# eriklindernoren/PyTorch-GAN

Hardware: NVIDIA H100
Metric: DCGAN 64x64 images/sec (full G+D step) (higher is better)
Workload: dtype tf32 (fp32 storage, fp32 accumulate)

## Files before the change

include/b200gan.h:

```cpp
#ifndef B200GAN_H
#define B200GAN_H

#include <stddef.h>
#include <stdint.h>

#ifdef __cplusplus
extern "C" {
#endif

#define B200GAN_VERSION 100

enum {
  B200GAN_OK = 0,
  B200GAN_E_UNSUPPORTED = -1,
  B200GAN_E_BAD_ARG = -2,
  B200GAN_E_CUDA = -3,
  B200GAN_E_ARCH = -4
};

enum { B200GAN_ACT_NONE = 0, B200GAN_ACT_LRELU = 1, B200GAN_ACT_RELU = 2, B200GAN_ACT_TANH = 3,
       B200GAN_ACT_SIGMOID = 4 };

enum { B200GAN_ALGO_AUTO = 0,
       B200GAN_ALGO_SIMT = 1,
       B200GAN_ALGO_TC = 2 };

enum { B200GAN_PAD_ZERO = 0, B200GAN_PAD_REFLECT = 1 };

enum {
  B200GAN_PACK_SIMT_FPROP = 0,
  B200GAN_PACK_SIMT_DGRAD = 1,
  B200GAN_PACK_TC_FPROP = 2,
  B200GAN_PACK_TC_DGRAD = 3,
  B200GAN_PACK_TC_FPROP_UP2 = 4,
  B200GAN_PACK_TC_DGRAD_UP2 = 5
};

typedef struct b200gan_conv_geom {
  int32_t N, H, W, C;
  int32_t K;
  int32_t R, S;
  int32_t stride;
  int32_t pad_t, pad_l, pad_b, pad_r;
  int32_t pad_mode;
  int32_t up;
  int32_t transposed;
  int32_t P, Q;
} b200gan_conv_geom;

typedef struct b200gan_epilogue {
  const float *bias;
  int32_t act;
  float slope;
  const float *chan_scale;
  double *stats;
  int32_t stats_per_sample;
  int32_t round_tf32;
} b200gan_epilogue;

int b200gan_version(void);
const char *b200gan_last_error(void);
int b200gan_check_device(void);

size_t b200gan_packed_weight_floats(const b200gan_conv_geom *g, int pack);
int b200gan_pack_weights(const b200gan_conv_geom *g, int pack, const float *w, float *packed,
                         void *stream);

typedef struct b200gan_pack_job {
  const float *w;
  float *packed;
  b200gan_conv_geom geom;
  int32_t pack;
} b200gan_pack_job;
int b200gan_pack_weights_multi(const b200gan_pack_job *jobs, int32_t count, void *stream);

int b200gan_conv2d_supported(const b200gan_conv_geom *g, int pass, int algo);

int b200gan_conv2d_fprop(const b200gan_conv_geom *g, const b200gan_epilogue *ep, const float *x,
                         const float *packed, float *y, int algo, void *stream);

size_t b200gan_conv2d_dgrad_workspace_floats(const b200gan_conv_geom *g, int algo);
int b200gan_conv2d_dgrad(const b200gan_conv_geom *g, const float *dy, const float *packed,
                         float *dx, float *workspace, int algo, void *stream);

size_t b200gan_conv2d_wgrad_workspace_floats(const b200gan_conv_geom *g, int algo);
int b200gan_conv2d_wgrad(const b200gan_conv_geom *g, const float *x, const float *dy, float *dw,
                         float *db, float *workspace, int algo, void *stream);
int b200gan_conv2d_wgrad_fused_bias(const b200gan_conv_geom *g, const float *x, const float *dy, float *dw,
                                    float *db, float *workspace, int algo, void *stream);

int b200gan_epilogue_bwd(const float *dy, const float *y, const float *chan_scale, int32_t act,
                         float slope, int64_t n, int32_t K, int64_t PQ, int32_t round_tf32,
                         float *dz, void *stream);

int b200gan_bias_grad(const float *dy, const float *y, const float *chan_scale, int32_t act, float slope,
                      int64_t rows, int32_t K, int64_t PQ, float *db, void *stream);

typedef struct b200gan_norm_desc {
  int32_t N, HW, C;
  int32_t per_sample;
  float eps;
  float momentum;
  int32_t act;
  float slope;
  int32_t round_tf32;
} b200gan_norm_desc;

int b200gan_norm_stats(const b200gan_norm_desc *d, const float *x, double *stats, void *stream);
int b200gan_norm_finalize(const b200gan_norm_desc *d, double *stats, const float *gamma,
                          const float *beta, float *mean_rstd, float *scale_shift,
                          float *running_mean, float *running_var, int64_t *num_batches_tracked,
                          void *stream);
int b200gan_norm_apply(const b200gan_norm_desc *d, const float *x, const float *scale_shift,
                       float *y, void *stream);
int b200gan_norm_bwd(const b200gan_norm_desc *d, const float *dy, const float *x, const float *y,
                     const float *mean_rstd, const float *scale_shift, const float *gamma, double *sums, float *dx,
                     float *dgamma_dbeta, void *stream);

int b200gan_conv2d_dgrad_norm_supported(const b200gan_conv_geom *g);
int b200gan_conv2d_dgrad_norm(const b200gan_conv_geom *g, const b200gan_norm_desc *d, const float *dy,
                              const float *packed, const float *x, const float *mean_rstd, const float *scale_shift,
                              double *sums, float *dx, void *stream);
int b200gan_norm_bwd_from_sums(const b200gan_norm_desc *d, const float *dy, const float *x, const float *mean_rstd,
                               const float *scale_shift, const float *gamma, double *sums, float *dx,
                               float *dgamma_dbeta, void *stream);

typedef struct b200gan_tail_desc {
  int32_t N, H, W, C;
  int32_t K;
  int32_t act_mid;
  float slope;
  int32_t act_out;
} b200gan_tail_desc;
int b200gan_tail_supported(const b200gan_tail_desc *d);
int b200gan_tail_fprop(const b200gan_tail_desc *d, const float *a, const float *scale_shift, const float *w,
                       const float *bias, float *out, void *stream);
size_t b200gan_tail_bwd_workspace_bytes(const b200gan_tail_desc *d);
int b200gan_tail_bwd(const b200gan_tail_desc *d, const float *a, const float *mean_rstd, const float *scale_shift,
                     const float *w, const float *g, void *workspace, float *da, float *dgamma_dbeta, float *dw,
                     float *db, int32_t round_tf32, void *stream);

int b200gan_nchw_to_nhwc(const float *x, float *y, int32_t N, int32_t C, int32_t HW, void *stream);
int b200gan_nhwc_to_nchw(const float *x, float *y, int32_t N, int32_t C, int32_t HW, void *stream);
int b200gan_upsample2x_fwd(const float *x, float *y, int32_t N, int32_t H, int32_t W, int32_t C,
                           void *stream);
int b200gan_upsample2x_bwd(const float *dy, float *dx, int32_t N, int32_t H, int32_t W, int32_t C,
                           void *stream);
int b200gan_pad2d_fwd(const float *x, float *y, int32_t N, int32_t H, int32_t W, int32_t C,
                      int32_t pad_t, int32_t pad_l, int32_t pad_b, int32_t pad_r, int32_t mode,
                      int32_t round_tf32, void *stream);
int b200gan_pad2d_bwd(const float *dy, float *dx, int32_t N, int32_t H, int32_t W, int32_t C,
                      int32_t pad_t, int32_t pad_l, int32_t pad_b, int32_t pad_r, int32_t mode,
                      void *stream);
int b200gan_act_fwd(const float *x, const float *mask, int32_t mask_per_channel, int32_t act,
                    float slope, int64_t n, int32_t C, int64_t HW, float *y, void *stream);

typedef struct b200gan_mlp_critic_desc {
  int32_t N, Din, H1, H2;
  float slope;
} b200gan_mlp_critic_desc;
int b200gan_mlp_critic_fwd(const b200gan_mlp_critic_desc *d, const float *x, const float *W1,
                           const float *b1, const float *W2, const float *b2, const float *W3,
                           const float *b3, float *out, float *m1, float *a1, float *m2, float *a2,
                           void *stream);
size_t b200gan_mlp_critic_bwd_workspace_floats(const b200gan_mlp_critic_desc *d);
int b200gan_mlp_critic_bwd(const b200gan_mlp_critic_desc *d, const float *dout, const float *x,
                           const float *W1, const float *W2, const float *W3, const float *m1,
                           const float *a1, const float *m2, const float *a2, float *dx, float *dW1,
                           float *db1, float *dW2, float *db2, float *dW3, float *db3, float *U1,
                           float *U2, float *workspace, void *stream);
size_t b200gan_mlp_critic_dbwd_workspace_floats(const b200gan_mlp_critic_desc *d);
int b200gan_mlp_critic_dbwd(const b200gan_mlp_critic_desc *d, const float *u, const float *dout,
// ... 85 lines not shown
```

pytorch-gan_b200/b200gan/_lib.py:

```python
import ctypes
import os

_HERE = os.path.dirname(os.path.abspath(__file__))
LIB_PATH = os.path.join(_HERE, "libb200gan.so")

c_i32, c_i64, c_f32, c_f64 = ctypes.c_int32, ctypes.c_int64, ctypes.c_float, ctypes.c_double
c_vp, c_sz = ctypes.c_void_p, ctypes.c_size_t

ACT_NONE, ACT_LRELU, ACT_RELU, ACT_TANH, ACT_SIGMOID = 0, 1, 2, 3, 4
ALGO_AUTO, ALGO_SIMT, ALGO_TC = 0, 1, 2
PAD_ZERO, PAD_REFLECT = 0, 1
PACK_SIMT_FPROP, PACK_SIMT_DGRAD, PACK_TC_FPROP, PACK_TC_DGRAD, PACK_TC_FPROP_UP2, PACK_TC_DGRAD_UP2 = range(6)


class ConvGeom(ctypes.Structure):
    _fields_ = [(n, c_i32) for n in (
        "N", "H", "W", "C", "K", "R", "S", "stride", "pad_t", "pad_l", "pad_b", "pad_r",
        "pad_mode", "up", "transposed", "P", "Q")]

    def key(self):
        return tuple(getattr(self, n) for n, _ in self._fields_)


class Epilogue(ctypes.Structure):
    _fields_ = [("bias", c_vp), ("act", c_i32), ("slope", c_f32), ("chan_scale", c_vp),
                ("stats", c_vp), ("stats_per_sample", c_i32), ("round_tf32", c_i32)]


class NormDesc(ctypes.Structure):
    _fields_ = [("N", c_i32), ("HW", c_i32), ("C", c_i32), ("per_sample", c_i32), ("eps", c_f32),
                ("momentum", c_f32), ("act", c_i32), ("slope", c_f32), ("round_tf32", c_i32)]


class MlpCriticDesc(ctypes.Structure):
    _fields_ = [("N", c_i32), ("Din", c_i32), ("H1", c_i32), ("H2", c_i32), ("slope", c_f32)]


MLP_GEN_MAX_LAYERS, MLP_GEN_MAX_WIDTH, MLP_GEN_MAX_N = 8, 8192, 8192


class MlpGenDesc(ctypes.Structure):
    _fields_ = [("L", c_i32), ("N", c_i32), ("width", c_i32 * (MLP_GEN_MAX_LAYERS + 1)),
                ("has_norm", c_i32 * MLP_GEN_MAX_LAYERS), ("slope", c_f32), ("eps", c_f32), ("momentum", c_f32)] + [
        (n, c_vp * MLP_GEN_MAX_LAYERS)
        for n in ("W", "b", "gamma", "beta", "running_mean", "running_var", "num_batches_tracked")]


class MlpGenGrads(ctypes.Structure):
    _fields_ = [(n, c_vp * MLP_GEN_MAX_LAYERS) for n in ("dW", "db", "dgamma", "dbeta")]


class PackJob(ctypes.Structure):
    _fields_ = [("w", c_vp), ("packed", c_vp), ("geom", ConvGeom), ("pack", c_i32)]


class NbBn(ctypes.Structure):
    _fields_ = [("stats", c_vp), ("gamma", c_vp), ("beta", c_vp), ("eps", c_f32), ("count", c_f64), ("groups", c_i32),
                ("reserved", c_i32)]


class TailDesc(ctypes.Structure):
    _fields_ = [("N", c_i32), ("H", c_i32), ("W", c_i32), ("C", c_i32), ("K", c_i32), ("act_mid", c_i32),
                ("slope", c_f32), ("act_out", c_i32)]


class AdamTensor(ctypes.Structure):
    _fields_ = [("p", c_vp), ("g", c_vp), ("m", c_vp), ("v", c_vp), ("n", c_i64)]


_P = ctypes.POINTER
SIGNATURES = {
    "b200gan_version": (c_i32, []),
    "b200gan_last_error": (ctypes.c_char_p, []),
    "b200gan_check_device": (c_i32, []),
    "b200gan_packed_weight_floats": (c_sz, [_P(ConvGeom), c_i32]),
    "b200gan_pack_weights": (c_i32, [_P(ConvGeom), c_i32, c_vp, c_vp, c_vp]),
    "b200gan_pack_weights_multi": (c_i32, [_P(PackJob), c_i32, c_vp]),
    "b200gan_conv2d_supported": (c_i32, [_P(ConvGeom), c_i32, c_i32]),
    "b200gan_conv2d_fprop": (c_i32, [_P(ConvGeom), _P(Epilogue), c_vp, c_vp, c_vp, c_i32, c_vp]),
    "b200gan_conv2d_dgrad_workspace_floats": (c_sz, [_P(ConvGeom), c_i32]),
    "b200gan_conv2d_dgrad": (c_i32, [_P(ConvGeom), c_vp, c_vp, c_vp, c_vp, c_i32, c_vp]),
    "b200gan_conv2d_wgrad_workspace_floats": (c_sz, [_P(ConvGeom), c_i32]),
    "b200gan_conv2d_wgrad": (c_i32, [_P(ConvGeom), c_vp, c_vp, c_vp, c_vp, c_vp, c_i32, c_vp]),
    "b200gan_conv2d_wgrad_fused_bias": (c_i32, [_P(ConvGeom), c_vp, c_vp, c_vp, c_vp, c_vp, c_i32, c_vp]),
    "b200gan_epilogue_bwd": (c_i32, [c_vp, c_vp, c_vp, c_i32, c_f32, c_i64, c_i32, c_i64, c_i32, c_vp, c_vp]),
    "b200gan_bias_grad": (c_i32, [c_vp, c_vp, c_vp, c_i32, c_f32, c_i64, c_i32, c_i64, c_vp, c_vp]),
    "b200gan_norm_stats": (c_i32, [_P(NormDesc), c_vp, c_vp, c_vp]),
    "b200gan_norm_finalize": (c_i32, [_P(NormDesc), c_vp, c_vp, c_vp, c_vp, c_vp, c_vp, c_vp, c_vp, c_vp]),
    "b200gan_norm_apply": (c_i32, [_P(NormDesc), c_vp, c_vp, c_vp, c_vp]),
    "b200gan_norm_bwd": (c_i32, [_P(NormDesc), c_vp, c_vp, c_vp, c_vp, c_vp, c_vp, c_vp, c_vp, c_vp, c_vp]),
    "b200gan_conv2d_dgrad_norm_supported": (c_i32, [_P(ConvGeom)]),
    "b200gan_conv2d_dgrad_norm": (c_i32, [_P(ConvGeom), _P(NormDesc)] + [c_vp] * 8),
    "b200gan_norm_bwd_from_sums": (c_i32, [_P(NormDesc)] + [c_vp] * 9),
    "b200gan_tail_supported": (c_i32, [_P(TailDesc)]),
    "b200gan_tail_fprop": (c_i32, [_P(TailDesc), c_vp, c_vp, c_vp, c_vp, c_vp, c_vp]),
    "b200gan_tail_bwd_workspace_bytes": (c_sz, [_P(TailDesc)]),
    "b200gan_tail_bwd": (c_i32, [_P(TailDesc)] + [c_vp] * 10 + [c_i32, c_vp]),
    "b200gan_nchw_to_nhwc": (c_i32, [c_vp, c_vp, c_i32, c_i32, c_i32, c_vp]),
    "b200gan_nhwc_to_nchw": (c_i32, [c_vp, c_vp, c_i32, c_i32, c_i32, c_vp]),
    "b200gan_upsample2x_fwd": (c_i32, [c_vp, c_vp, c_i32, c_i32, c_i32, c_i32, c_vp]),
    "b200gan_upsample2x_bwd": (c_i32, [c_vp, c_vp, c_i32, c_i32, c_i32, c_i32, c_vp]),
    "b200gan_pad2d_fwd": (c_i32, [c_vp, c_vp] + [c_i32] * 10 + [c_vp]),
    "b200gan_pad2d_bwd": (c_i32, [c_vp, c_vp] + [c_i32] * 9 + [c_vp]),
    "b200gan_act_fwd": (c_i32, [c_vp, c_vp, c_i32, c_i32, c_f32, c_i64, c_i32, c_i64, c_vp, c_vp]),
    "b200gan_mlp_critic_fwd": (c_i32, [_P(MlpCriticDesc)] + [c_vp] * 13),
    "b200gan_mlp_critic_bwd_workspace_floats": (c_sz, [_P(MlpCriticDesc)]),
    "b200gan_mlp_critic_bwd": (c_i32, [_P(MlpCriticDesc)] + [c_vp] * 20),
    "b200gan_mlp_critic_dbwd_workspace_floats": (c_sz, [_P(MlpCriticDesc)]),
    "b200gan_mlp_critic_dbwd": (c_i32, [_P(MlpCriticDesc)] + [c_vp] * 15),
    "b200gan_critic_step_workspace_floats": (c_sz, [_P(MlpCriticDesc)]),
    "b200gan_critic_step_mlp": (c_i32, [_P(MlpCriticDesc), c_f32] + [c_vp] * 18),
    "b200gan_mlp_gen_saved_floats": (c_sz, [_P(MlpGenDesc)]),
    "b200gan_mlp_gen_workspace_floats": (c_sz, [_P(MlpGenDesc)]),
    "b200gan_mlp_gen_fwd": (c_i32, [_P(MlpGenDesc)] + [c_vp] * 5),
    "b200gan_mlp_gen_bwd": (c_i32, [_P(MlpGenDesc)] + [c_vp] * 5 + [_P(MlpGenGrads), c_vp, c_vp]),
    "b200gan_nb_supported": (c_i32, [_P(ConvGeom)]),
    "b200gan_nb_groups_supported": (c_i32, [_P(ConvGeom), c_i32]),
    "b200gan_nb_fprop": (c_i32, [_P(ConvGeom), _P(NbBn), c_vp, c_vp, c_vp, c_f32, c_vp, c_vp, c_vp, c_i32, c_f32, c_vp,
                                 c_vp, c_vp, c_i32, c_vp]),
    "b200gan_nb_dz": (c_i32, [c_i32, c_i64, c_i32, c_vp, c_vp, c_vp, c_i32, c_f32, _P(NbBn), c_vp, c_vp, c_vp, c_vp]),
    "b200gan_nb_wgrad_workspace_floats": (c_sz, [_P(ConvGeom)]),
    "b200gan_nb_wgrad": (c_i32, [_P(ConvGeom), _P(NbBn), c_vp, c_vp, c_vp, c_vp, c_vp]),
    "b200gan_nb_dgrad": (c_i32, [_P(ConvGeom), c_vp, c_vp, _P(NbBn), c_vp, c_vp, c_vp, c_vp]),
    "b200gan_nb_tail_fwd": (c_i32, [c_i32, c_i32, c_i32, _P(NbBn), c_vp, c_vp, c_vp, c_f32, c_vp, c_vp, c_i32, c_vp]),
    "b200gan_nb_tail_bwd": (c_i32, [c_i32, c_i32, c_i32, _P(NbBn), c_vp, c_vp, c_i32, c_vp, c_vp, c_vp]),
    "b200gan_linear1_fwd": (c_i32, [c_vp, c_vp, c_vp, c_vp, c_i32, c_i32, c_i32, c_vp]),
    "b200gan_linear1_bwd": (c_i32, [c_vp] * 7 + [c_i32, c_i32, c_i32, c_vp]),
    "b200gan_bce_fwd": (c_i32, [c_vp, c_vp, c_vp, c_i64, c_vp]),
    "b200gan_bce_bwd": (c_i32, [c_vp, c_vp, c_vp, c_vp, c_i64, c_vp]),
    "b200gan_adam_multi": (c_i32, [_P(AdamTensor), c_i32, c_f64, c_f64, c_f64, c_f64, c_f32, c_vp, c_vp]),
}

_lib = None


def load():
    global _lib
    if _lib is not None:
        return _lib
    if not os.path.exists(LIB_PATH):
        raise RuntimeError(
            f"{LIB_PATH} is missing: run `python pytorch-gan_b200/build.py` (or __graft_entry__.build()). "
            "b200gan has no CPU / cuDNN fallback.")
    lib = ctypes.CDLL(LIB_PATH)
    for name, (res, args) in SIGNATURES.items():
        fn = getattr(lib, name)
        fn.restype = res
        fn.argtypes = args
    _lib = lib
    return lib


CALLS = 0


def check(rc, what=""):
    global CALLS
    CALLS += 1
    if rc != 0:
        msg = load().b200gan_last_error().decode("utf-8", "replace")
        raise RuntimeError(f"libb200gan {what} failed (code {rc}): {msg}")
```

pytorch-gan_b200/csrc/wgrad_tc.cu:

```cuda
#include "tc_common.cuh"
#include <stdlib.h>

namespace b200gan {

constexpr int WG_THREADS = 384;
constexpr int WG_MAX_JOBS = 52;
constexpr int WG_PIX = 32;
constexpr int WG_CHUNK_BYTES = WG_PIX * 128;

struct WgJob {
  int16_t s_dc, d_dc;
  int8_t s_da, d_da;
  int8_t s_dw, s_dh;
  int8_t db;
  int8_t pad_;
};

struct WgParams {
  WgJob jobs[WG_MAX_JOBS];
  int32_t njobs;
  int32_t bw_log2, bh_log2;
  int32_t tiles_w, tiles_h, N;
  int32_t imgs_per_box;
  int32_t tiles_total, tiles_per_split;
  int32_t s_is_a;
  int32_t mtiles, ntiles;
  int32_t ldn;
  int32_t mtotal;
  float *partial;
  float *db;
};

template <int NB, int STAGES>
struct WgSmem {
  static constexpr int A_BYTES = 4 * WG_CHUNK_BYTES;
  static constexpr int B_BYTES = (NB / 32) * WG_CHUNK_BYTES;
  static constexpr int STAGE_BYTES = A_BYTES + B_BYTES;
  static constexpr int RING = STAGES * STAGE_BYTES;
  static constexpr int T_BYTES = NB * 128;
  static constexpr int STAGING = (NB / 32) * 16384;
  static constexpr int MAIN = RING + 2 * T_BYTES > STAGING ? RING + 2 * T_BYTES : STAGING;
  static constexpr int TOTAL = MAIN + 1024 + 256;
  static_assert(TOTAL <= 232448, "wgrad_tc_kernel: shared memory");
};

__device__ __forceinline__ void wg_consumers_sync() { asm volatile("bar.sync 1, 256;" ::: "memory"); }

__device__ __forceinline__ int wg_kpos(int p) { return (p & ~7) | ((p & 7) >> 1) | ((p & 1) << 2); }

template <int NB, int STAGES>
__global__ void __launch_bounds__(WG_THREADS, 1)
wgrad_tc_kernel(const __grid_constant__ CUtensorMap tmX, const __grid_constant__ CUtensorMap tmY,
                const __grid_constant__ CUtensorMap tmP, const __grid_constant__ WgParams p) {
  using L = WgSmem<NB, STAGES>;
  extern __shared__ uint8_t smem_raw[];
  uint8_t *smem = reinterpret_cast<uint8_t *>((reinterpret_cast<uintptr_t>(smem_raw) + 1023) & ~(uintptr_t)1023);
  uint64_t *full = reinterpret_cast<uint64_t *>(smem + L::MAIN);
  uint64_t *empty = full + STAGES;

  const int warp = threadIdx.x >> 5, lane = threadIdx.x & 31;
  const int split = blockIdx.x, job = blockIdx.y;
  const int mt = blockIdx.z / p.ntiles, nt = blockIdx.z % p.ntiles;
  const int t_begin = split * p.tiles_per_split;
  int t_end = t_begin + p.tiles_per_split;
  if (t_end > p.tiles_total) t_end = p.tiles_total;
  const int iters = t_end - t_begin;

  if (threadIdx.x == 0) {
    tma_prefetch_desc(&tmX);
    tma_prefetch_desc(&tmY);
    for (int s = 0; s < STAGES; ++s) {
      mbar_init(&full[s], 1);
      mbar_init(&empty[s], 256);
    }
    fence_barrier_init();
  }
  __syncthreads();

  if (warp < 4) {
    setmaxnreg_dec<40>();
    if (warp == 0 && lane == 0) {
      const WgJob jb = p.jobs[job];
      const CUtensorMap *mapA = p.s_is_a ? &tmX : &tmY;
      const CUtensorMap *mapB = p.s_is_a ? &tmY : &tmX;
      const int a_dc = p.s_is_a ? jb.s_dc : jb.d_dc, a_da = p.s_is_a ? jb.s_da : jb.d_da;
      const int a_dw = p.s_is_a ? jb.s_dw : 0, a_dh = p.s_is_a ? jb.s_dh : 0;
      const int b_dc = p.s_is_a ? jb.d_dc : jb.s_dc, b_da = p.s_is_a ? jb.d_da : jb.s_da;
      const int b_dw = p.s_is_a ? 0 : jb.s_dw, b_dh = p.s_is_a ? 0 : jb.s_dh;
      int stage = 0;
      uint32_t phase = 0;
      for (int it = 0; it < iters; ++it) {
        int t = t_begin + it;
        const int tw = t % p.tiles_w;
        t /= p.tiles_w;
        const int th = t % p.tiles_h;
        const int n = (t / p.tiles_h) * p.imgs_per_box;
        const int w0 = tw << p.bw_log2, h0 = th << p.bh_log2;
        mbar_wait(&empty[stage], phase ^ 1);
        uint8_t *sa = smem + stage * L::STAGE_BYTES;
        uint8_t *sb = sa + L::A_BYTES;
        mbar_arrive_expect_tx(&full[stage], L::STAGE_BYTES);
#pragma unroll
        for (int c = 0; c < 4; ++c)
          tma_load_5d(sa + c * WG_CHUNK_BYTES, mapA, &full[stage], a_dc + (mt * 4 + c) * 32, w0 + a_dw, a_da,
                      h0 + a_dh, n);
#pragma unroll
        for (int c = 0; c < NB / 32; ++c)
          tma_load_5d(sb + c * WG_CHUNK_BYTES, mapB, &full[stage], b_dc + (nt * (NB / 32) + c) * 32, w0 + b_dw, b_da,
                      h0 + b_dh, n);
        if (++stage == STAGES) {
          stage = 0;
          phase ^= 1;
        }
      }
    }
  } else {
    setmaxnreg_inc<232>();
    if (iters == 0) return;
    const int ct = threadIdx.x - 128;
    const int half = ct >> 7;
    const int tp = ct & 31, tq = ct >> 5;
    const int tk = wg_kpos(tp);
    const int wq = tq & 3;
    const int ac = 16 * (wq & 1) + (lane >> 2), ap = 2 * (lane & 3);
    const int abase = (2 * half + (wq >> 1)) * WG_CHUNK_BYTES + ap * 128 + (ac & 3) * 4;
    const uint32_t aoff[4] = {
        (uint32_t)(abase + ((((ac >> 2)) ^ ap) << 4)),
        (uint32_t)(abase + ((((ac >> 2) + 2) ^ ap) << 4)),
        (uint32_t)(abase + 128 + ((((ac >> 2)) ^ (ap + 1)) << 4)),
        (uint32_t)(abase + 128 + ((((ac >> 2) + 2) ^ (ap + 1)) << 4))};
    float acc[NB / 2];
    const bool db_job = p.db != nullptr && p.jobs[job].db;
    const bool dbA = db_job && !p.s_is_a && nt == 0;
    const bool dbB = db_job && p.s_is_a && mt == 0;
    float dsa0 = 0.f, dsa1 = 0.f;
    float dsb[NB <= 64 ? NB / 8 : 1];
#pragma unroll
    for (int i = 0; i < (NB <= 64 ? NB / 8 : 1); ++i) dsb[i] = 0.f;
    int stage = 0;
    uint32_t phase = 0;
    auto prepare = [&](int it, uint32_t(&fa)[16]) {
      uint8_t *tb = smem + L::RING + (it & 1) * L::T_BYTES;
      mbar_wait(&full[stage], phase);
      wg_consumers_sync();
      const uint8_t *src = smem + stage * L::STAGE_BYTES;
#pragma unroll
      for (int k = 0; k < WG_PIX / 8; ++k)
#pragma unroll
        for (int j = 0; j < 4; ++j) fa[4 * k + j] = *reinterpret_cast<const uint32_t *>(src + aoff[j] + k * 1024);
      if (dbA) {
#pragma unroll
        for (int k = 0; k < WG_PIX / 8; ++k) {
          dsa0 += __uint_as_float(fa[4 * k]) + __uint_as_float(fa[4 * k + 2]);
          dsa1 += __uint_as_float(fa[4 * k + 1]) + __uint_as_float(fa[4 * k + 3]);
        }
      }
#pragma unroll
      for (int c = 0; c < NB / 32; ++c) {
        const float4 v = *reinterpret_cast<const float4 *>(src + L::A_BYTES + c * WG_CHUNK_BYTES + tp * 128 +
                                                           ((tq ^ (tp & 7)) << 4));
        const float e[4] = {v.x, v.y, v.z, v.w};
        if constexpr (NB <= 64) {
          if (dbB) {
#pragma unroll
            for (int i = 0; i < 4; ++i) dsb[4 * c + i] += e[i];
          }
        }
#pragma unroll
        for (int i = 0; i < 4; ++i) {
          const int r = c * 32 + tq * 4 + i;
          *reinterpret_cast<float *>(tb + r * 128 + (((tk >> 2) ^ (r & 7)) << 4) + (tk & 3) * 4) = e[i];
        }
      }
      mbar_arrive(&empty[stage]);
      fence_proxy_async();
      wg_consumers_sync();
      if (++stage == STAGES) {
        stage = 0;
        phase ^= 1;
      }
    };
    auto mma = [&](int it, const uint32_t(&fa)[16]) {
      const uint32_t sb = smem_u32(smem + L::RING + (it & 1) * L::T_BYTES);
      wgmma_fence();
#pragma unroll
      for (int k = 0; k < WG_PIX / 8; ++k)
        wgmma_tf32_rs<NB>(acc, fa + 4 * k, gmma_desc_sw128(sb + k * 32), (it > 0 || k > 0) ? 1u : 0u);
      wgmma_commit();
    };
    uint32_t fa0[16], fa1[16];
    prepare(0, fa0);
#pragma unroll 1
    for (int it = 0; it < iters; it += 2) {
      mma(it, fa0);
      if (it + 1 < iters) prepare(it + 1, fa1);
      wgmma_wait<0>();
      if (it + 1 < iters) {
        mma(it + 1, fa1);
        if (it + 2 < iters) prepare(it + 2, fa0);
        wgmma_wait<0>();
      }
    }
    wgmma_wait<0>();
    wgmma_fence_regs<NB / 2>(acc);
    if (dbA) {
      dsa0 += __shfl_xor_sync(0xffffffffu, dsa0, 1);
      dsa1 += __shfl_xor_sync(0xffffffffu, dsa1, 1);
      dsa0 += __shfl_xor_sync(0xffffffffu, dsa0, 2);
      dsa1 += __shfl_xor_sync(0xffffffffu, dsa1, 2);
      if ((lane & 3) == 0) {
        const int ch = (mt * 4 + 2 * half + (wq >> 1)) * 32 + ac;
        atomicAdd(p.db + ch, dsa0);
        atomicAdd(p.db + ch + 8, dsa1);
      }
    }
    if constexpr (NB <= 64) {
      if (dbB) {
#pragma unroll
        for (int i = 0; i < NB / 8; ++i) {
          float s = dsb[i];
#pragma unroll
          for (int o = 16; o > 0; o >>= 1) s += __shfl_xor_sync(0xffffffffu, s, o);
          if (lane == 0) atomicAdd(p.db + nt * NB + (i >> 2) * 32 + tq * 4 + (i & 3), s);
        }
      }
    }
    wg_consumers_sync();
    store_acc_sw128<NB>(smem, acc, half * 64);
    fence_proxy_async();
    wg_consumers_sync();
    if (ct == 0) {
      const int row0 = job * p.mtotal + mt * 128;
#pragma unroll 1
      for (int c = 0; c < NB; c += 32) tma_reduce_add_2d(&tmP, smem + (c >> 5) * 16384, nt * NB + c, row0);
      tma_store_commit_and_wait_read();
    }
  }
}

struct WgReduceP {
  int32_t K, C, R, S, njobs, s_is_a, up2, transposed;
  int32_t mtotal, ldn;
};
__device__ __forceinline__ bool up2_contrib(int r, int a, int d) {
  if (a == 0) return d == 0 ? r == 0 : r >= 1;
  return d == 0 ? r <= 1 : r == 2;
}
__global__ void wgrad_reduce_kernel(const float *__restrict__ partial, float *__restrict__ dw, WgReduceP p) {
  int64_t total = (int64_t)p.K * p.C * p.R * p.S;
  for (int64_t i = (int64_t)blockIdx.x * blockDim.x + threadIdx.x; i < total;
       i += (int64_t)gridDim.x * blockDim.x) {
    int c = (int)(i % p.C);
    int64_t t = i / p.C;
    int k = (int)(t % p.K);
    t /= p.K;
    int s = (int)(t % p.S), r = (int)(t / p.S);
    const int sch = p.transposed ? k : c;
    const int dch = p.transposed ? c : k;
    int64_t elem = p.s_is_a ? (int64_t)sch * p.ldn + dch : (int64_t)dch * p.ldn + sch;
    int64_t job_stride = (int64_t)p.mtotal * p.ldn;
    const float *base = partial + elem;
    float acc = 0.f;
    if (!p.up2) {
      acc = __ldg(base + (int64_t)(r * p.S + s) * job_stride);
    } else {
      for (int j = 0; j < 16; ++j) {
        int ph = j >> 2, tp = j & 3;
        if (up2_contrib(r, ph >> 1, tp >> 1) && up2_contrib(s, ph & 1, tp & 1)) acc += __ldg(base + j * job_stride);
      }
    }
    const int64_t o = p.transposed ? (((int64_t)c * p.K + k) * p.R + r) * p.S + s
                                   : (((int64_t)k * p.C + c) * p.R + r) * p.S + s;
    dw[o] = acc;
  }
}


constexpr int WR_COL = 32, WR_ROW = 8, WR_TAPS = 16;
__global__ void __launch_bounds__(256)
wgrad_reduce_tile_kernel(const float *__restrict__ partial, float *__restrict__ dw, WgReduceP p) {
  __shared__ float s[WR_ROW][WR_COL][WR_TAPS + 1];
  const int RS = p.R * p.S;
  const int tin = p.up2 ? 16 : RS;
  const bool col_is_k = (p.s_is_a != 0) != (p.transposed != 0);
  const int ncol = col_is_k ? p.K : p.C, nrow = col_is_k ? p.C : p.K;
  const int tiles_col = (ncol + WR_COL - 1) / WR_COL;
  const int col0 = (blockIdx.x % tiles_col) * WR_COL, row0 = (blockIdx.x / tiles_col) * WR_ROW;
  const int64_t job_stride = (int64_t)p.mtotal * p.ldn;
  const int tid = threadIdx.x;
  for (int e = tid; e < WR_COL * WR_ROW * tin; e += 256) {
    const int cl = e % WR_COL, rw = (e / WR_COL) % WR_ROW, j = e / (WR_COL * WR_ROW);
    float v = 0.f;
    if (col0 + cl < ncol && row0 + rw < nrow) v = __ldg(partial + j * job_stride + (int64_t)(row0 + rw) * p.ldn + col0 + cl);
    s[rw][cl][j] = v;
  }
  __syncthreads();
  const bool col_is_b = col_is_k == (p.transposed != 0);
  const int nb = p.transposed ? p.K : p.C;
  for (int e = tid; e < WR_COL * WR_ROW * RS; e += 256) {
    const int t = e % RS;
    int cl, rw;
    if (col_is_b) { cl = (e / RS) % WR_COL; rw = e / (RS * WR_COL); }
    else          { rw = (e / RS) % WR_ROW; cl = e / (RS * WR_ROW); }
    const int col = col0 + cl, row = row0 + rw;
    if (col >= ncol || row >= nrow) continue;
    float acc;
    if (!p.up2) {
      acc = s[rw][cl][t];
    } else {
      const int r = t / 3, q = t % 3;
      acc = 0.f;
#pragma unroll
      for (int j = 0; j < 16; ++j) {
        const int ph = j >> 2, tp = j & 3;
        if (up2_contrib(r, ph >> 1, tp >> 1) && up2_contrib(q, ph & 1, tp & 1)) acc += s[rw][cl][j];
      }
    }
    const int a = col_is_b ? row : col, b = col_is_b ? col : row;
    dw[((int64_t)a * nb + b) * RS + t] = acc;
  }
}

static int ilog2c(int v) {
  int l = 0;
  while ((1 << l) < v) ++l;
  return l;
}

struct WgPlan {
  int s_is_a, NB, mtiles, ntiles, mtotal, ldn, njobs, bwl, bhl, tiles_w, tiles_h, tiles_total, nsplits, tps, Ho, Wo;
  int sch, dch;
  int ipb;
};

static bool wg_plan(const b200gan_conv_geom *g, WgPlan &pl) {
  if (g->pad_mode != B200GAN_PAD_ZERO || g->N < 1) return false;
  if (g->stride != 1 && g->stride != 2) return false;
  if (g->C % 32 || g->K % 32 || 2 * g->C > 32767 || 2 * g->K > 32767) return false;
  const bool up2 = g->up == 2;
  if (up2 && (g->transposed || g->stride != 1 ||
              !(g->R == 3 && g->S == 3 && g->pad_t == 1 && g->pad_l == 1 && g->pad_b == 1 && g->pad_r == 1)))
    return false;
  if (g->R * g->S > WG_MAX_JOBS || g->R > 15 || g->S > 15 || g->pad_t > 15 || g->pad_l > 15) return false;
  pl.sch = g->transposed ? g->K : g->C;
  pl.dch = g->transposed ? g->C : g->K;
  if (g->stride == 2) {
    const int Hf = g->transposed ? g->P : g->H, Wf = g->transposed ? g->Q : g->W;
    if ((Hf & 1) || (Wf & 1)) return false;
  }
  if (pl.dch % 128 == 0) pl.s_is_a = 0;
  else if (pl.sch % 128 == 0) pl.s_is_a = 1;
  else return false;
  const int mch = pl.s_is_a ? pl.sch : pl.dch, nch = pl.s_is_a ? pl.dch : pl.sch;
  pl.NB = nch % 128 == 0 ? 128 : (nch % 64 == 0 ? 64 : 32);
  if (nch % 256 == 0) pl.NB = 256;
  pl.mtotal = mch;
  pl.ldn = nch;
  pl.mtiles = mch / 128;
  pl.ntiles = nch / pl.NB;
  pl.njobs = up2 ? 16 : g->R * g->S;
  pl.Ho = up2 ? g->H : (g->transposed ? g->H : g->P);
  pl.Wo = up2 ? g->W : (g->transposed ? g->W : g->Q);
  const int pl2 = 5;
  pl.bwl = ilog2c(pl.Wo);
  if (pl.bwl > pl2) pl.bwl = pl2;
  pl.bhl = ilog2c(pl.Ho);
  if (pl.bhl > pl2 - pl.bwl) pl.bhl = pl2 - pl.bwl;
  pl.tiles_w = ceil_div(pl.Wo, 1 << pl.bwl);
  pl.tiles_h = ceil_div(pl.Ho, 1 << pl.bhl);
  pl.ipb = WG_PIX >> (pl.bwl + pl.bhl);
  int64_t tt = (int64_t)ceil_div(g->N, pl.ipb) * pl.tiles_w * pl.tiles_h;
  if (tt > (1 << 30)) return false;
  pl.tiles_total = (int)tt;
  const int64_t ctas_per_split = (int64_t)pl.njobs * pl.mtiles * pl.ntiles;
  int max_ns = pl.tiles_total / 8;
  if (max_ns < 1) max_ns = 1;
  if (max_ns > 4 * num_sms()) max_ns = 4 * num_sms();
  int ns = 1;
  int64_t best = -1;
  for (int s = 1; s <= max_ns; ++s) {
    const int64_t waves = ceil_div64(s * ctas_per_split, num_sms());
    const int64_t cost = waves * (ceil_div(pl.tiles_total, s) + 8);
    if (best < 0 || cost < best) {
      best = cost;
      ns = s;
    }
  }
  pl.tps = ceil_div(pl.tiles_total, ns);
  pl.nsplits = ceil_div(pl.tiles_total, pl.tps);
  return true;
}

int tc_wgrad_supported(const b200gan_conv_geom *g) {
  WgPlan pl;
  return wg_plan(g, pl) ? 1 : 0;
}

size_t tc_wgrad_workspace_floats(const b200gan_conv_geom *g) {
  WgPlan pl;
  if (!wg_plan(g, pl)) return 0;
  return (size_t)pl.njobs * pl.mtotal * pl.ldn;
}

template <int NB, int STAGES>
static int launch_wg(const CUtensorMap &tmX, const CUtensorMap &tmY, const CUtensorMap &tmP, const WgParams &p, dim3 grid,
                     cudaStream_t st) {
  constexpr int SMEM = WgSmem<NB, STAGES>::TOTAL;
  static std::atomic<uint64_t> attr_done{0};
  if (int e = ensure_dynamic_smem(wgrad_tc_kernel<NB, STAGES>, SMEM, attr_done)) return e;
  wgrad_tc_kernel<NB, STAGES><<<grid, WG_THREADS, SMEM, st>>>(tmX, tmY, tmP, p);
  B2_LAUNCH_CHECK();
  return B200GAN_OK;
}

int tc_wgrad(const b200gan_conv_geom *g, const float *x, const float *dy, float *dw, float *db, float *ws,
             cudaStream_t st) {
  WgPlan pl;
  if (!wg_plan(g, pl)) B2_UNSUPPORTED("tensor-core wgrad: geometry not supported");
  B2_CHECK_ARG(ws != nullptr, "tensor-core wgrad: workspace required");
  B2_CHECK_ARG(!(db && g->transposed), "tensor-core wgrad: bias gradient of a ConvTranspose2d is not fused");
  B2_CHECK_ARG(((uintptr_t)x % 16 == 0) && ((uintptr_t)dy % 16 == 0) && ((uintptr_t)ws % 16 == 0),
               "tensor-core wgrad: pointers must be 16-byte aligned");
  const bool up2 = g->up == 2;
  const int st2 = g->stride == 2;
  WgParams p;
  memset(&p, 0, sizeof(p));
  p.njobs = pl.njobs;
  if (up2) {
    for (int ph = 0; ph < 4; ++ph)
      for (int tp = 0; tp < 4; ++tp) {
        int a = ph >> 1, b = ph & 1, dr = tp >> 1, ds = tp & 1;
        WgJob &j = p.jobs[ph * 4 + tp];
        j.d_dc = (int16_t)(b * g->K); j.d_da = (int8_t)a; j.s_dh = (int8_t)(a - 1 + dr); j.s_dw = (int8_t)(b - 1 + ds);
        j.db = tp == 0;
      }
  } else {
    p.jobs[0].db = 1;
    for (int r = 0; r < g->R; ++r)
      for (int s2 = 0; s2 < g->S; ++s2) {
        WgJob &j = p.jobs[r * g->S + s2];
        const int eh = r - g->pad_t, ew = s2 - g->pad_l;
        if (!st2) {
          j.s_dh = (int8_t)eh; j.s_dw = (int8_t)ew;
        } else {
          j.s_dh = (int8_t)(eh >= 0 ? eh / 2 : -((-eh + 1) / 2)); j.s_da = (int8_t)(eh & 1);
          j.s_dw = (int8_t)(ew >= 0 ? ew / 2 : -((-ew + 1) / 2)); j.s_dc = (int16_t)((ew & 1) * pl.sch);
        }
      }
  }
  p.bw_log2 = pl.bwl; p.bh_log2 = pl.bhl;
  p.tiles_w = pl.tiles_w; p.tiles_h = pl.tiles_h; p.N = g->N; p.imgs_per_box = pl.ipb;
  p.tiles_total = pl.tiles_total; p.tiles_per_split = pl.tps;
  p.s_is_a = pl.s_is_a; p.mtiles = pl.mtiles; p.ntiles = pl.ntiles; p.ldn = pl.ldn; p.mtotal = pl.mtotal;
  p.partial = ws;
  p.db = db;

  const float *sptr = g->transposed ? dy : x, *dptr = g->transposed ? x : dy;
  const uint64_t Hs = g->transposed ? g->P : g->H, Ws = g->transposed ? g->Q : g->W, Cs = pl.sch;
  const uint64_t Hd = g->transposed ? g->H : g->P, Wd = g->transposed ? g->W : g->Q, Cd = pl.dch;
  CUtensorMap tmX, tmY;
  const uint32_t box[5] = {32, (uint32_t)(1 << pl.bwl), 1, (uint32_t)(1 << pl.bhl), (uint32_t)pl.ipb};
  {
    uint64_t dims[5], strides[4];
    if (!st2) {
      dims[0] = Cs; dims[1] = Ws; dims[2] = 1; dims[3] = Hs; dims[4] = g->N;
      strides[0] = Cs * 4; strides[1] = Ws * Cs * 4; strides[2] = Ws * Cs * 4; strides[3] = Hs * Ws * Cs * 4;
    } else {
      dims[0] = 2 * Cs; dims[1] = Ws / 2; dims[2] = 2; dims[3] = Hs / 2; dims[4] = g->N;
      strides[0] = 2 * Cs * 4; strides[1] = Ws * Cs * 4; strides[2] = 2 * Ws * Cs * 4; strides[3] = Hs * Ws * Cs * 4;
    }
    if (int e = make_tmap_f32(&tmX, sptr, 5, dims, strides, box)) return e;
  }
  {
    uint64_t dims[5], strides[4];
    if (!up2) {
      dims[0] = Cd; dims[1] = Wd; dims[2] = 1; dims[3] = Hd; dims[4] = g->N;
      strides[0] = Cd * 4; strides[1] = Wd * Cd * 4; strides[2] = Wd * Cd * 4; strides[3] = Hd * Wd * Cd * 4;
    } else {
      dims[0] = 2 * Cd; dims[1] = Wd / 2; dims[2] = 2; dims[3] = Hd / 2; dims[4] = g->N;
      strides[0] = 2 * Cd * 4; strides[1] = Wd * Cd * 4; strides[2] = 2 * Wd * Cd * 4; strides[3] = Hd * Wd * Cd * 4;
    }
    if (int e = make_tmap_f32(&tmY, dptr, 5, dims, strides, box)) return e;
  }
  CUtensorMap tmP;
  {
    uint64_t dims[2] = {(uint64_t)pl.ldn, (uint64_t)pl.njobs * pl.mtotal};
    uint64_t strides[1] = {(uint64_t)pl.ldn * 4};
    uint32_t pbox[2] = {32, 128};
    if (int e = make_tmap_f32(&tmP, ws, 2, dims, strides, pbox)) return e;
  }
  B2_CUDA(cudaMemsetAsync(ws, 0, (size_t)pl.njobs * pl.mtotal * pl.ldn * sizeof(float), st));
  if (db) B2_CUDA(cudaMemsetAsync(db, 0, (size_t)g->K * sizeof(float), st));
  dim3 grid((unsigned)pl.nsplits, (unsigned)pl.njobs, (unsigned)(pl.mtiles * pl.ntiles));
  int rc = pl.NB == 256 ? launch_wg<256, 3>(tmX, tmY, tmP, p, grid, st)
           : pl.NB == 128 ? launch_wg<128, 6>(tmX, tmY, tmP, p, grid, st)
           : pl.NB == 64 ? launch_wg<64, 8>(tmX, tmY, tmP, p, grid, st)
                         : launch_wg<32, 8>(tmX, tmY, tmP, p, grid, st);
  if (rc) return rc;
  WgReduceP rp;
  rp.K = g->K; rp.C = g->C; rp.R = g->R; rp.S = g->S; rp.njobs = pl.njobs;
  rp.s_is_a = pl.s_is_a; rp.up2 = up2 ? 1 : 0; rp.transposed = g->transposed ? 1 : 0; rp.mtotal = pl.mtotal; rp.ldn = pl.ldn;
  int64_t total = (int64_t)g->K * g->C * g->R * g->S;
  if (g->R * g->S <= WR_TAPS && g->K >= 32 && g->C >= 32) {
    const bool col_is_k = (pl.s_is_a != 0) != (g->transposed != 0);
    const int ncol = col_is_k ? g->K : g->C, nrow = col_is_k ? g->C : g->K;
    const unsigned tiles = (unsigned)(ceil_div(ncol, WR_COL) * ceil_div(nrow, WR_ROW));
    wgrad_reduce_tile_kernel<<<tiles, 256, 0, st>>>(ws, dw, rp);
    B2_LAUNCH_CHECK();
    return B200GAN_OK;
  }
  unsigned blocks = (unsigned)(ceil_div64(total, 256) > num_sms() * 16 ? num_sms() * 16 : ceil_div64(total, 256));
  wgrad_reduce_kernel<<<blocks, 256, 0, st>>>(ws, dw, rp);
  B2_LAUNCH_CHECK();
  return B200GAN_OK;
}

}
```

Before: 49030.

## Group upsample-conv wgrad phase jobs into paired wide-N tensor-core CTAs

For upsample-by-2 convolutions with small channel counts, the weight-gradient kernel now pairs phase/tap jobs that share the same source shift into one CTA with a doubled N tile. Each such CTA loads the source tile once and computes two output slots, while corner jobs run alone with their own split length. A new grouped split planner balances pair and single job lengths across SMs. This cuts redundant source-tile TMA loads and the job count, at the cost of more complex slot indexing, a larger NB template instance, and uneven per-CTA work. New plan and job-mask entry points are exposed as well.

Result: faster. 49830, median of 6 (+1.6%).

```diff
diff --git a/include/b200gan.h b/include/b200gan.h
--- a/include/b200gan.h
+++ b/include/b200gan.h
@@ -88,6 +88,9 @@
                          float *db, float *workspace, int algo, void *stream);
 int b200gan_conv2d_wgrad_fused_bias(const b200gan_conv_geom *g, const float *x, const float *dy, float *dw,
                                     float *db, float *workspace, int algo, void *stream);
+int b200gan_tc_wgrad_plan(const b200gan_conv_geom *g, int32_t sms, int32_t *out);
+int b200gan_tc_wgrad_jobs(const b200gan_conv_geom *g, const float *x, const float *dy, float *dw, float *workspace,
+                          int32_t grouped, uint32_t job_mask, void *stream);
 
 int b200gan_epilogue_bwd(const float *dy, const float *y, const float *chan_scale, int32_t act,
                          float slope, int64_t n, int32_t K, int64_t PQ, int32_t round_tf32,
diff --git a/pytorch-gan_b200/b200gan/_lib.py b/pytorch-gan_b200/b200gan/_lib.py
--- a/pytorch-gan_b200/b200gan/_lib.py
+++ b/pytorch-gan_b200/b200gan/_lib.py
@@ -83,6 +83,8 @@
     "b200gan_conv2d_wgrad_workspace_floats": (c_sz, [_P(ConvGeom), c_i32]),
     "b200gan_conv2d_wgrad": (c_i32, [_P(ConvGeom), c_vp, c_vp, c_vp, c_vp, c_vp, c_i32, c_vp]),
     "b200gan_conv2d_wgrad_fused_bias": (c_i32, [_P(ConvGeom), c_vp, c_vp, c_vp, c_vp, c_vp, c_i32, c_vp]),
+    "b200gan_tc_wgrad_plan": (c_i32, [_P(ConvGeom), c_i32, _P(c_i32)]),
+    "b200gan_tc_wgrad_jobs": (c_i32, [_P(ConvGeom), c_vp, c_vp, c_vp, c_vp, c_i32, ctypes.c_uint32, c_vp]),
     "b200gan_epilogue_bwd": (c_i32, [c_vp, c_vp, c_vp, c_i32, c_f32, c_i64, c_i32, c_i64, c_i32, c_vp, c_vp]),
     "b200gan_bias_grad": (c_i32, [c_vp, c_vp, c_vp, c_i32, c_f32, c_i64, c_i32, c_i64, c_vp, c_vp]),
     "b200gan_norm_stats": (c_i32, [_P(NormDesc), c_vp, c_vp, c_vp]),
diff --git a/pytorch-gan_b200/csrc/wgrad_tc.cu b/pytorch-gan_b200/csrc/wgrad_tc.cu
--- a/pytorch-gan_b200/csrc/wgrad_tc.cu
+++ b/pytorch-gan_b200/csrc/wgrad_tc.cu
@@ -13,7 +13,9 @@
   int8_t s_da, d_da;
   int8_t s_dw, s_dh;
   int8_t db;
-  int8_t pad_;
+  int8_t slot;
+  int16_t d_dc2;
+  int8_t d_da2, slot2;
 };
 
 struct WgParams {
@@ -23,7 +25,9 @@
   int32_t tiles_w, tiles_h, N;
   int32_t imgs_per_box;
   int32_t tiles_total, tiles_per_split;
+  int32_t tiles_per_split1;
   int32_t s_is_a;
+  int32_t pairs;
   int32_t mtiles, ntiles;
   int32_t ldn;
   int32_t mtotal;
@@ -61,10 +65,12 @@
   const int warp = threadIdx.x >> 5, lane = threadIdx.x & 31;
   const int split = blockIdx.x, job = blockIdx.y;
   const int mt = blockIdx.z / p.ntiles, nt = blockIdx.z % p.ntiles;
-  const int t_begin = split * p.tiles_per_split;
-  int t_end = t_begin + p.tiles_per_split;
+  const bool single = p.pairs && p.jobs[job].slot2 < 0;
+  const int tps = single ? p.tiles_per_split1 : p.tiles_per_split;
+  const int t_begin = split * tps;
+  int t_end = t_begin + tps;
   if (t_end > p.tiles_total) t_end = p.tiles_total;
-  const int iters = t_end - t_begin;
+  const int iters = t_end > t_begin ? t_end - t_begin : 0;
 
   if (threadIdx.x == 0) {
     tma_prefetch_desc(&tmX);
@@ -99,15 +105,19 @@
         mbar_wait(&empty[stage], phase ^ 1);
         uint8_t *sa = smem + stage * L::STAGE_BYTES;
         uint8_t *sb = sa + L::A_BYTES;
-        mbar_arrive_expect_tx(&full[stage], L::STAGE_BYTES);
+        mbar_arrive_expect_tx(&full[stage], single ? L::A_BYTES + L::B_BYTES / 2 : L::STAGE_BYTES);
 #pragma unroll
         for (int c = 0; c < 4; ++c)
           tma_load_5d(sa + c * WG_CHUNK_BYTES, mapA, &full[stage], a_dc + (mt * 4 + c) * 32, w0 + a_dw, a_da,
                       h0 + a_dh, n);
 #pragma unroll
-        for (int c = 0; c < NB / 32; ++c)
-          tma_load_5d(sb + c * WG_CHUNK_BYTES, mapB, &full[stage], b_dc + (nt * (NB / 32) + c) * 32, w0 + b_dw, b_da,
-                      h0 + b_dh, n);
+        for (int c = 0; c < NB / 32; ++c) {
+          const bool second = p.pairs && c >= NB / 64;
+          if (second && single) break;
+          tma_load_5d(sb + c * WG_CHUNK_BYTES, mapB, &full[stage], second ? jb.d_dc2 + (c - NB / 64) * 32
+                                                                          : b_dc + (nt * (NB / 32) + c) * 32,
+                      w0 + b_dw, second ? jb.d_da2 : b_da, h0 + b_dh, n);
+        }
         if (++stage == STAGES) {
           stage = 0;
           phase ^= 1;
@@ -134,9 +144,11 @@
     const bool dbA = db_job && !p.s_is_a && nt == 0;
     const bool dbB = db_job && p.s_is_a && mt == 0;
     float dsa0 = 0.f, dsa1 = 0.f;
-    float dsb[NB <= 64 ? NB / 8 : 1];
-#pragma unroll
-    for (int i = 0; i < (NB <= 64 ? NB / 8 : 1); ++i) dsb[i] = 0.f;
+    constexpr int DBN = NB <= 64 ? NB : (NB == 128 ? 64 : 0);
+    const int bchunks = single ? NB / 64 : NB / 32;
+    float dsb[DBN ? DBN / 8 : 1];
+#pragma unroll
+    for (int i = 0; i < (DBN ? DBN / 8 : 1); ++i) dsb[i] = 0.f;
     int stage = 0;
     uint32_t phase = 0;
     auto prepare = [&](int it, uint32_t(&fa)[16]) {
@@ -157,11 +169,12 @@
       }
 #pragma unroll
       for (int c = 0; c < NB / 32; ++c) {
+        if (c >= bchunks) break;
         const float4 v = *reinterpret_cast<const float4 *>(src + L::A_BYTES + c * WG_CHUNK_BYTES + tp * 128 +
                                                            ((tq ^ (tp & 7)) << 4));
         const float e[4] = {v.x, v.y, v.z, v.w};
-        if constexpr (NB <= 64) {
-          if (dbB) {
+        if constexpr (DBN > 0) {
+          if (dbB && c < DBN / 32) {
 #pragma unroll
             for (int i = 0; i < 4; ++i) dsb[4 * c + i] += e[i];
           }
@@ -214,10 +227,11 @@
         atomicAdd(p.db + ch + 8, dsa1);
       }
     }
-    if constexpr (NB <= 64) {
+    if constexpr (DBN > 0) {
       if (dbB) {
 #pragma unroll
-        for (int i = 0; i < NB / 8; ++i) {
+        for (int i = 0; i < DBN / 8; ++i) {
+          if ((i >> 2) >= bchunks) break;
           float s = dsb[i];
 #pragma unroll
           for (int o = 16; o > 0; o >>= 1) s += __shfl_xor_sync(0xffffffffu, s, o);
@@ -230,9 +244,11 @@
     fence_proxy_async();
     wg_consumers_sync();
     if (ct == 0) {
-      const int row0 = job * p.mtotal + mt * 128;
+      const WgJob &jb = p.jobs[job];
+      const int nw = p.pairs ? NB / 2 : NB;
 #pragma unroll 1
-      for (int c = 0; c < NB; c += 32) tma_reduce_add_2d(&tmP, smem + (c >> 5) * 16384, nt * NB + c, row0);
+      for (int c = 0; c < (single ? nw : NB); c += 32)
+        tma_reduce_add_2d(&tmP, smem + (c >> 5) * 16384, nt * nw + c % nw, (c < nw ? jb.slot : jb.slot2) * p.mtotal + mt * 128);
       tma_store_commit_and_wait_read();
     }
   }
@@ -331,9 +347,54 @@
   int s_is_a, NB, mtiles, ntiles, mtotal, ldn, njobs, bwl, bhl, tiles_w, tiles_h, tiles_total, nsplits, tps, Ho, Wo;
   int sch, dch;
   int ipb;
+  int grouped, ljobs, pair_nsplits, pair_tps;
 };
-
-static bool wg_plan(const b200gan_conv_geom *g, WgPlan &pl) {
+constexpr int WG_PAIR_JOBS = 6;
+
+static void wg_split(int tiles_total, int64_t ctas_per_split, int sms, int &nsplits, int &tps) {
+  int max_ns = tiles_total / 8;
+  if (max_ns < 1) max_ns = 1;
+  if (max_ns > 4 * sms) max_ns = 4 * sms;
+  int ns = 1;
+  int64_t best = -1;
+  for (int s = 1; s <= max_ns; ++s) {
+    const int64_t waves = ceil_div64(s * ctas_per_split, sms);
+    const int64_t cost = waves * (ceil_div(tiles_total, s) + 8);
+    if (best < 0 || cost < best) {
+      best = cost;
+      ns = s;
+    }
+  }
+  tps = ceil_div(tiles_total, ns);
+  nsplits = ceil_div(tiles_total, tps);
+}
+
+static void wg_split_grouped(WgPlan &pl, int sms) {
+  const int64_t T = pl.tiles_total, w2 = 128 + 2 * pl.dch, w1 = 128 + pl.dch;
+  int max_ns = pl.tiles_total / 8;
+  if (max_ns < 1) max_ns = 1;
+  if (max_ns > 4 * sms) max_ns = 4 * sms;
+  const int64_t min_waves = ceil_div64((int64_t)(WG_PAIR_JOBS + pl.ljobs) * pl.mtiles, sms);
+  int64_t best = -1;
+  for (int s2 = 1; s2 <= max_ns; ++s2) {
+    const int64_t len2 = ceil_div64(T, s2);
+    int s1 = (int)ceil_div64(T * w1, len2 * w2);
+    if (s1 < 1) s1 = 1;
+    while (s1 < max_ns && ceil_div64(T, s1) * w1 > len2 * w2) ++s1;
+    const int64_t waves = ceil_div64((int64_t)(WG_PAIR_JOBS * s2 + pl.ljobs * s1) * pl.mtiles, sms);
+    if (waves > min_waves) continue;
+    const int64_t cost = waves * (len2 + 8);
+    if (best < 0 || cost < best) {
+      best = cost;
+      pl.pair_tps = (int)len2;
+      pl.tps = (int)ceil_div64(T, s1);
+    }
+  }
+  pl.pair_nsplits = ceil_div(pl.tiles_total, pl.pair_tps);
+  pl.nsplits = ceil_div(pl.tiles_total, pl.tps);
+}
+
+static bool wg_plan(const b200gan_conv_geom *g, WgPlan &pl, int sms) {
   if (g->pad_mode != B200GAN_PAD_ZERO || g->N < 1) return false;
   if (g->stride != 1 && g->stride != 2) return false;
   if (g->C % 32 || g->K % 32 || 2 * g->C > 32767 || 2 * g->K > 32767) return false;
@@ -372,33 +433,22 @@
   int64_t tt = (int64_t)ceil_div(g->N, pl.ipb) * pl.tiles_w * pl.tiles_h;
   if (tt > (1 << 30)) return false;
   pl.tiles_total = (int)tt;
-  const int64_t ctas_per_split = (int64_t)pl.njobs * pl.mtiles * pl.ntiles;
-  int max_ns = pl.tiles_total / 8;
-  if (max_ns < 1) max_ns = 1;
-  if (max_ns > 4 * num_sms()) max_ns = 4 * num_sms();
-  int ns = 1;
-  int64_t best = -1;
-  for (int s = 1; s <= max_ns; ++s) {
-    const int64_t waves = ceil_div64(s * ctas_per_split, num_sms());
-    const int64_t cost = waves * (ceil_div(pl.tiles_total, s) + 8);
-    if (best < 0 || cost < best) {
-      best = cost;
-      ns = s;
-    }
-  }
-  pl.tps = ceil_div(pl.tiles_total, ns);
-  pl.nsplits = ceil_div(pl.tiles_total, pl.tps);
+  pl.grouped = up2 && pl.s_is_a && nch <= 64;
+  pl.ljobs = pl.grouped ? 4 : pl.njobs;
+  pl.pair_nsplits = pl.pair_tps = 0;
+  if (pl.grouped) wg_split_grouped(pl, sms);
+  else wg_split(pl.tiles_total, (int64_t)pl.ljobs * pl.mtiles * pl.ntiles, sms, pl.nsplits, pl.tps);
   return true;
 }
 
 int tc_wgrad_supported(const b200gan_conv_geom *g) {
   WgPlan pl;
-  return wg_plan(g, pl) ? 1 : 0;
+  return wg_plan(g, pl, num_sms()) ? 1 : 0;
 }
 
 size_t tc_wgrad_workspace_floats(const b200gan_conv_geom *g) {
   WgPlan pl;
-  if (!wg_plan(g, pl)) return 0;
+  if (!wg_plan(g, pl, num_sms())) return 0;
   return (size_t)pl.njobs * pl.mtotal * pl.ldn;
 }
 
@@ -413,32 +463,78 @@
   return B200GAN_OK;
 }
 
-int tc_wgrad(const b200gan_conv_geom *g, const float *x, const float *dy, float *dw, float *db, float *ws,
-             cudaStream_t st) {
+static int launch_wg_nb(int NB, const CUtensorMap &tmX, const CUtensorMap &tmY, const CUtensorMap &tmP,
+                        const WgParams &p, dim3 grid, cudaStream_t st) {
+  return NB == 256 ? launch_wg<256, 3>(tmX, tmY, tmP, p, grid, st)
+         : NB == 128 ? launch_wg<128, 6>(tmX, tmY, tmP, p, grid, st)
+         : NB == 64 ? launch_wg<64, 8>(tmX, tmY, tmP, p, grid, st)
+                    : launch_wg<32, 8>(tmX, tmY, tmP, p, grid, st);
+}
+
+static int tc_wgrad_run(const b200gan_conv_geom *g, const float *x, const float *dy, float *dw, float *db, float *ws,
+                        int grouped, uint32_t job_mask, cudaStream_t st) {
   WgPlan pl;
-  if (!wg_plan(g, pl)) B2_UNSUPPORTED("tensor-core wgrad: geometry not supported");
+  if (!wg_plan(g, pl, num_sms())) B2_UNSUPPORTED("tensor-core wgrad: geometry not supported");
   B2_CHECK_ARG(ws != nullptr, "tensor-core wgrad: workspace required");
   B2_CHECK_ARG(!(db && g->transposed), "tensor-core wgrad: bias gradient of a ConvTranspose2d is not fused");
   B2_CHECK_ARG(((uintptr_t)x % 16 == 0) && ((uintptr_t)dy % 16 == 0) && ((uintptr_t)ws % 16 == 0),
                "tensor-core wgrad: pointers must be 16-byte aligned");
   const bool up2 = g->up == 2;
   const int st2 = g->stride == 2;
+  if (grouped == 0 && pl.grouped) {
+    pl.grouped = 0;
+    pl.ljobs = pl.njobs;
+    wg_split(pl.tiles_total, (int64_t)pl.ljobs * pl.mtiles * pl.ntiles, num_sms(), pl.nsplits, pl.tps);
+  }
   WgParams p;
   memset(&p, 0, sizeof(p));
-  p.njobs = pl.njobs;
-  if (up2) {
+  if (pl.grouped) {
+    WgJob corners[4] = {};
+    int nc = 0;
+    for (int dh = -1; dh <= 1; ++dh)
+      for (int dw2 = -1; dw2 <= 1; ++dw2) {
+        int ph[4], nph = 0;
+        for (int a = 0; a < 2; ++a)
+          for (int b = 0; b < 2; ++b)
+            if (dh - a + 1 >= 0 && dh - a + 1 <= 1 && dw2 - b + 1 >= 0 && dw2 - b + 1 <= 1) ph[nph++] = 2 * a + b;
+        auto fill = [&](WgJob &j, int q) {
+          const int a = q >> 1, b = q & 1;
+          j.s_dh = (int8_t)dh; j.s_dw = (int8_t)dw2;
+          j.d_dc = (int16_t)(b * g->K); j.d_da = (int8_t)a;
+          j.slot = (int8_t)(4 * q + 2 * (dh - a + 1) + (dw2 - b + 1));
+        };
+        if (nph == 1) {
+          WgJob &j = corners[nc++];
+          fill(j, ph[0]);
+          j.slot2 = -1;
+          j.db = 1;
+        } else {
+          for (int i = 0; i < nph; i += 2) {
+            WgJob &j = p.jobs[p.njobs++];
+            WgJob second;
+            fill(j, ph[i]);
+            fill(second, ph[i + 1]);
+            j.d_dc2 = second.d_dc; j.d_da2 = second.d_da; j.slot2 = second.slot;
+          }
+        }
+      }
+    for (int i = 0; i < nc; ++i) p.jobs[p.njobs++] = corners[i];
+    p.pairs = 1;
+  } else if (up2) {
     for (int ph = 0; ph < 4; ++ph)
       for (int tp = 0; tp < 4; ++tp) {
+        if (!(job_mask >> (ph * 4 + tp) & 1)) continue;
         int a = ph >> 1, b = ph & 1, dr = tp >> 1, ds = tp & 1;
-        WgJob &j = p.jobs[ph * 4 + tp];
+        WgJob &j = p.jobs[p.njobs++];
         j.d_dc = (int16_t)(b * g->K); j.d_da = (int8_t)a; j.s_dh = (int8_t)(a - 1 + dr); j.s_dw = (int8_t)(b - 1 + ds);
         j.db = tp == 0;
+        j.slot = (int8_t)(ph * 4 + tp);
       }
   } else {
-    p.jobs[0].db = 1;
     for (int r = 0; r < g->R; ++r)
       for (int s2 = 0; s2 < g->S; ++s2) {
-        WgJob &j = p.jobs[r * g->S + s2];
+        if (r * g->S + s2 < 32 && !(job_mask >> (r * g->S + s2) & 1)) continue;
+        WgJob &j = p.jobs[p.njobs++];
         const int eh = r - g->pad_t, ew = s2 - g->pad_l;
         if (!st2) {
           j.s_dh = (int8_t)eh; j.s_dw = (int8_t)ew;
@@ -446,14 +542,20 @@
           j.s_dh = (int8_t)(eh >= 0 ? eh / 2 : -((-eh + 1) / 2)); j.s_da = (int8_t)(eh & 1);
           j.s_dw = (int8_t)(ew >= 0 ? ew / 2 : -((-ew + 1) / 2)); j.s_dc = (int16_t)((ew & 1) * pl.sch);
         }
+        j.db = r == 0 && s2 == 0;
+        j.slot = (int8_t)(r * g->S + s2);
       }
   }
   p.bw_log2 = pl.bwl; p.bh_log2 = pl.bhl;
   p.tiles_w = pl.tiles_w; p.tiles_h = pl.tiles_h; p.N = g->N; p.imgs_per_box = pl.ipb;
-  p.tiles_total = pl.tiles_total; p.tiles_per_split = pl.tps;
+  p.tiles_total = pl.tiles_total;
   p.s_is_a = pl.s_is_a; p.mtiles = pl.mtiles; p.ntiles = pl.ntiles; p.ldn = pl.ldn; p.mtotal = pl.mtotal;
   p.partial = ws;
   p.db = db;
+  if (!pl.grouped && p.njobs != pl.ljobs)
+    wg_split(pl.tiles_total, (int64_t)p.njobs * pl.mtiles * pl.ntiles, num_sms(), pl.nsplits, pl.tps);
+  p.tiles_per_split = pl.grouped ? pl.pair_tps : pl.tps;
+  p.tiles_per_split1 = pl.tps;
 
   const float *sptr = g->transposed ? dy : x, *dptr = g->transposed ? x : dy;
   const uint64_t Hs = g->transposed ? g->P : g->H, Ws = g->transposed ? g->Q : g->W, Cs = pl.sch;
@@ -491,12 +593,14 @@
   }
   B2_CUDA(cudaMemsetAsync(ws, 0, (size_t)pl.njobs * pl.mtotal * pl.ldn * sizeof(float), st));
   if (db) B2_CUDA(cudaMemsetAsync(db, 0, (size_t)g->K * sizeof(float), st));
-  dim3 grid((unsigned)pl.nsplits, (unsigned)pl.njobs, (unsigned)(pl.mtiles * pl.ntiles));
-  int rc = pl.NB == 256 ? launch_wg<256, 3>(tmX, tmY, tmP, p, grid, st)
-           : pl.NB == 128 ? launch_wg<128, 6>(tmX, tmY, tmP, p, grid, st)
-           : pl.NB == 64 ? launch_wg<64, 8>(tmX, tmY, tmP, p, grid, st)
-                         : launch_wg<32, 8>(tmX, tmY, tmP, p, grid, st);
-  if (rc) return rc;
+  if (pl.grouped) {
+    dim3 grid((unsigned)(pl.pair_nsplits > pl.nsplits ? pl.pair_nsplits : pl.nsplits), (unsigned)p.njobs,
+              (unsigned)pl.mtiles);
+    if (int rc = launch_wg_nb(2 * pl.NB, tmX, tmY, tmP, p, grid, st)) return rc;
+  } else if (p.njobs) {
+    dim3 grid((unsigned)pl.nsplits, (unsigned)p.njobs, (unsigned)(pl.mtiles * pl.ntiles));
+    if (int rc = launch_wg_nb(pl.NB, tmX, tmY, tmP, p, grid, st)) return rc;
+  }
   WgReduceP rp;
   rp.K = g->K; rp.C = g->C; rp.R = g->R; rp.S = g->S; rp.njobs = pl.njobs;
   rp.s_is_a = pl.s_is_a; rp.up2 = up2 ? 1 : 0; rp.transposed = g->transposed ? 1 : 0; rp.mtotal = pl.mtotal; rp.ldn = pl.ldn;
@@ -515,4 +619,34 @@
   return B200GAN_OK;
 }
 
-}
+int tc_wgrad(const b200gan_conv_geom *g, const float *x, const float *dy, float *dw, float *db, float *ws,
+             cudaStream_t st) {
+  return tc_wgrad_run(g, x, dy, dw, db, ws, -1, 0xffffffffu, st);
+}
+
+}
+
+extern "C" int b200gan_tc_wgrad_plan(const b200gan_conv_geom *g, int32_t sms, int32_t *out) {
+  using namespace b200gan;
+  B2_CHECK_ARG(g && out && sms > 0, "tc_wgrad_plan: bad argument");
+  if (int e = validate_geom(g)) return e;
+  WgPlan pl;
+  if (!wg_plan(g, pl, sms)) B2_UNSUPPORTED("tc_wgrad_plan: geometry not supported");
+  const int32_t v[7] = {pl.grouped,
+                        pl.grouped ? 2 * pl.NB : pl.NB,
+                        pl.grouped ? (pl.pair_nsplits > pl.nsplits ? pl.pair_nsplits : pl.nsplits) : pl.nsplits,
+                        pl.grouped ? WG_PAIR_JOBS + pl.ljobs : pl.ljobs,
+                        pl.grouped ? pl.mtiles : pl.mtiles * pl.ntiles,
+                        pl.pair_nsplits,
+                        pl.nsplits};
+  for (int i = 0; i < 7; ++i) out[i] = v[i];
+  return B200GAN_OK;
+}
+
+extern "C" int b200gan_tc_wgrad_jobs(const b200gan_conv_geom *g, const float *x, const float *dy, float *dw,
+                                     float *workspace, int32_t grouped, uint32_t job_mask, void *stream) {
+  using namespace b200gan;
+  B2_CHECK_ARG(g && x && dy && dw, "tc_wgrad_jobs: null pointer");
+  if (int e = validate_geom(g)) return e;
+  return tc_wgrad_run(g, x, dy, dw, nullptr, workspace, grouped, job_mask, as_stream(stream));
+}
```
